# suvajit-patra/sl-hwgat

Measured on AMD Instinct MI355X. Metric: clips/sec fwd+bwd at B=64 T=128 J=67; %HBM roofline; 1->8 GPU scaling, higher is better.
Workload: dtype f32

## Files before the change

### sl-hwgat_amd/csrc/gemm_f32.h

```cpp
#pragma once
#include "common.h"

struct NtArgs {
    const float* A; const float* W; const float* bias; float* C;
    float* C2; const float* res; const float* aux;
    const float* mean; const float* rstd; const float* gamma; const float* beta;
    int64_t M; int N, K;
    uint32_t pro_seed, epi_seed; float pro_p, epi_p;
    int64_t row0;
    float* stat_sum; float* stat_sq;
    int mg_F, mg_K;
    const uint32_t* seed_base;
};

struct MergeWalk {
    int k, f; int64_t b; int F, K, step;
    __device__ __forceinline__ void start(int64_t m, int F_, int K_, int step_) {
        F = F_; K = K_; step = step_;
        const uint32_t mm = (uint32_t)m, fr = mm / (uint32_t)K_;
        k = (int)(mm - fr * (uint32_t)K_);
        const uint32_t bb = fr / (uint32_t)F_;
        f = (int)(fr - bb * (uint32_t)F_);
        b = bb;
    }
    __device__ __forceinline__ int64_t mrow() const { return (b * (F >> 1) + (f >> 1)) * K + k; }
    __device__ __forceinline__ int64_t off(int N) const { return mrow() * (2 * (int64_t)N) + (int64_t)(f & 1) * N; }
    __device__ __forceinline__ void next() {
        k += step;
        const bool wk = k >= K;
        k -= wk ? K : 0;
        f += wk ? 1 : 0;
        const bool wf = f >= F;
        f -= wf ? F : 0;
        b += wf ? 1 : 0;
    }
};

struct TnArgs {
    const float* A; const float* B; float* dW; float* db;
    const float* mean; const float* rstd; const float* gamma; const float* beta;
    int64_t M; int N, K;
    int n_split; int64_t rows_per_split;
    uint32_t pro_seed; float pro_p;
    int64_t row0;
    const uint32_t* seed_base;
    float* det_dw; float* det_db; int det_cap;
};


int hwgat_launch_tn256(TnArgs a, hipStream_t st, float* ws = nullptr, int64_t ws_floats = 0);
int64_t hwgat_tn256_ws_floats(int64_t M, int N, int K);

int hwgat_launch_nt256(const NtArgs& a, int pro, int epi, hipStream_t st);
```

### sl-hwgat_amd/csrc/gemm_f32.hip

```cpp
#include <stdlib.h>
#include <type_traits>
#include "common.h"
#include "fused_ops.h"
#include "gemm_f32.h"
#include "gemm_tn64.h"

namespace {

constexpr int BK_MIN = 16;

using NtSmall = TileCfg<2, 2, 2, 2>;
using NtBig = TileCfg<4, 2, 2, 4, 32, 1>;
using NtK16 = TileCfg<2, 2, 2, 2, 16, 3>;
using NtN64 = TileCfg<4, 1, 1, 2>;

template <int PRO, int EPI, typename C, bool RAGGED = false, int STAT = 0>
__global__ __launch_bounds__(C::THREADS, C::OCC * C::THREADS / 256) void gemm_nt_k(NtArgs p) {
    HWGAT_RESOLVE_SEEDS2(p);
    constexpr int BM = C::BM, BN = C::BN, TMW = C::TMW, TNW = C::TNW, PA = C::PA, PW = C::PW, RPP = C::RPP;
    constexpr int BK = C::BK, LDT = C::LDT;
    __shared__ __attribute__((aligned(16))) float sm[2 * (BM + BN) * LDT];
    const int tid = threadIdx.x, lane = tid & 63, wave = tid >> 6;
    const int lq = lane & 31, hh = lane >> 5;
    const int wm = wave / C::WN, wn = wave % C::WN;
    const int tiles_n = p.N / BN;
    const int row_blocks = RAGGED ? (int)((p.M + BM - 1) / BM) : (int)(p.M / BM);
    const int n_tiles = row_blocks * tiles_n;
    const int64_t m_last = p.M - 1;
    const int n_slab = p.K / BK;
    const int lrow = tid / C::TPR, lc4 = (tid % C::TPR) * 4;
    const uint32_t pro_th = drop_thresh(p.pro_p);
    const float pro_sc = 1.0f / (1.0f - p.pro_p);

    f32x4 ra[PA], rw[PW];
    float ln_mean[PA], ln_rstd[PA];
    f32x4 ln_g, ln_b;

    const int swz_tiles = (row_blocks / 8) * 8 * tiles_n;
    auto tile_origin = [&](int t, int64_t& m0, int& n0) {
        int rb, nt;
        if (t < swz_tiles) {
            rb = (t / (8 * tiles_n)) * 8 + (t & 7);
            nt = (t >> 3) % tiles_n;
        } else {
            const int w = t - swz_tiles;
            rb = (row_blocks / 8) * 8 + w / tiles_n;
            nt = w % tiles_n;
        }
        m0 = (int64_t)rb * BM;
        n0 = nt * BN;
    };
    auto issue = [&](int64_t m0, int n0, int slab, bool new_tile) {
        const int k0 = slab * BK + lc4;
#pragma unroll
        for (int i = 0; i < PA; ++i) {
            int64_t row = m0 + lrow + RPP * i;
            if constexpr (RAGGED) row = row < m_last ? row : m_last;
            ra[i] = *reinterpret_cast<const f32x4*>(p.A + row * p.K + k0);
            if constexpr (PRO == PRO_LN) {
                if (new_tile) { ln_mean[i] = p.mean[row]; ln_rstd[i] = p.rstd[row]; }
            }
        }
#pragma unroll
        for (int i = 0; i < PW; ++i)
            rw[i] = *reinterpret_cast<const f32x4*>(p.W + (int64_t)(n0 + lrow + RPP * i) * p.K + k0);
        if constexpr (PRO == PRO_LN) {
            ln_g = *reinterpret_cast<const f32x4*>(p.gamma + k0);
            ln_b = *reinterpret_cast<const f32x4*>(p.beta + k0);
        }
    };
    auto commit = [&](int buf, int64_t m0, int slab) {
        float* As = sm + buf * ((BM + BN) * LDT);
        float* Ws = As + BM * LDT;
        const int k0 = slab * BK + lc4;
#pragma unroll
        for (int i = 0; i < PA; ++i) {
            f32x4 a = ra[i];
            if constexpr (PRO == PRO_LN) {
                a = (a - ln_mean[i]) * (ln_rstd[i] * ln_g) + ln_b;
            } else if constexpr (PRO == PRO_DROP) {
                if (pro_th) a *= drop_keep4(p.pro_seed, (uint64_t)((RAGGED ? p.row0 : 0) + m0 + lrow + RPP * i) * p.K + k0, pro_th, pro_sc);
            }
            *reinterpret_cast<f32x4*>(As + (lrow + RPP * i) * LDT + lc4) = a;
        }
#pragma unroll
        for (int i = 0; i < PW; ++i) *reinterpret_cast<f32x4*>(Ws + (lrow + RPP * i) * LDT + lc4) = rw[i];
    };

    int t = blockIdx.x;
    if (t >= n_tiles) return;
    int64_t m0; int n0;
    tile_origin(t, m0, n0);
    issue(m0, n0, 0, true);
    commit(0, m0, 0);
    __syncthreads();
    int buf = 0;

    while (true) {
        f32x16 acc[TMW][TNW];
#pragma unroll
        for (int i = 0; i < TMW; ++i)
#pragma unroll
            for (int j = 0; j < TNW; ++j)
#pragma unroll
                for (int e = 0; e < 16; ++e) acc[i][j][e] = 0.f;

        int tn = t; int64_t mn = m0; int nn = n0;
        for (int s = 0; s < n_slab; ++s) {
            bool have_next = true, new_tile = false;
            int s_next = s + 1;
            if (s_next == n_slab) {
                tn = t + gridDim.x;
                have_next = tn < n_tiles;
                s_next = 0;
                new_tile = true;
                if (have_next) tile_origin(tn, mn, nn);
            }
            if (have_next) issue(mn, nn, s_next, new_tile);

            const float* As = sm + buf * ((BM + BN) * LDT);
            const float* Ws = As + BM * LDT;
            const float* ap = As + (wm * (TMW * 32) + lq) * LDT + 4 * hh;
            const float* wp = Ws + (wn * (TNW * 32) + lq) * LDT + 4 * hh;
#pragma unroll
            for (int kk = 0; kk < BK / 8; ++kk) {
                f32x4 af[TMW], bf[TNW];
#pragma unroll
                for (int i = 0; i < TMW; ++i) af[i] = *reinterpret_cast<const f32x4*>(ap + i * 32 * LDT + 8 * kk);
#pragma unroll
                for (int j = 0; j < TNW; ++j) bf[j] = *reinterpret_cast<const f32x4*>(wp + j * 32 * LDT + 8 * kk);
#pragma unroll
                for (int e = 0; e < 4; ++e)
#pragma unroll
                    for (int i = 0; i < TMW; ++i)
#pragma unroll
                        for (int j = 0; j < TNW; ++j)
                            acc[i][j] = __builtin_amdgcn_mfma_f32_32x32x2f32(af[i][e], bf[j][e], acc[i][j], 0, 0, 0);
            }
            if (have_next) commit(buf ^ 1, mn, s_next);
            __syncthreads();
            buf ^= 1;
        }

        {
            const uint32_t epi_th = drop_thresh(p.epi_p);
            const float epi_sc = 1.0f / (1.0f - p.epi_p);
            constexpr int SW = ((BM + BN) * LDT >= (C::THREADS / 64) * 32 * 68) ? 64 : 32;
            constexpr int SLD = SW + 4, LPR = SW / 4, RPS = 64 / LPR, NPS = 32 / RPS;
            float* stg = sm + (buf ^ 1) * ((BM + BN) * LDT) + wave * (32 * SLD);
            const int er = lane / LPR, ec = (lane % LPR) * 4;
            float* rowstat = sm + (buf ^ 1) * ((BM + BN) * LDT) + (C::THREADS / 64) * (32 * SLD);
            if constexpr (STAT == X_STAT || STAT == X_STAT_MERGE) {
                static_assert((C::THREADS / 64) * 32 * SLD + 2 * BM <= (BM + BN) * LDT, "no room for the row statistics");
                for (int q = tid; q < 2 * BM; q += C::THREADS) rowstat[q] = 0.f;
                __syncthreads();
            }
#pragma unroll
            for (int jc = 0; jc < TNW * 32 / SW; ++jc) {
                const int col = n0 + wn * (TNW * 32) + jc * SW + ec;
                f32x4 bv = {0.f, 0.f, 0.f, 0.f};
                if constexpr (epi_has_bias(EPI))
                    if (p.bias) bv = *reinterpret_cast<const f32x4*>(p.bias + col);
                f32x4 sv = bv, cv = bv;
                if constexpr (STAT == X_LNFOLD) {
                    sv = *reinterpret_cast<const f32x4*>(p.gamma + col);
                    cv = *reinterpret_cast<const f32x4*>(p.beta + col);
                }
#pragma unroll
                for (int i = 0; i < TMW; ++i) {
                    float rr_[NPS], rm[NPS];
                    if constexpr (STAT == X_LNFOLD) {
#pragma unroll
                        for (int ps = 0; ps < NPS; ++ps) {
                            int64_t grow = m0 + wm * (TMW * 32) + i * 32 + ps * RPS + er;
                            if constexpr (RAGGED) grow = grow < m_last ? grow : m_last;
                            rr_[ps] = p.rstd[grow]; rm[ps] = p.mean[grow];
                        }
                    }
                    MergeWalk mw;
                    if constexpr (STAT == X_STAT_MERGE) mw.start(m0 + wm * (TMW * 32) + i * 32 + er, p.mg_F, p.mg_K, RPS);
                    f32x4 ex[NPS];
                    if constexpr (epi_reads_extra(EPI)) {
                        const float* src = EPI == EPI_BIAS_DROP_RES ? p.res : p.aux;
#pragma unroll
                        for (int ps = 0; ps < NPS; ++ps) {
                            int64_t grow = m0 + wm * (TMW * 32) + i * 32 + ps * RPS + er;
                            if constexpr (RAGGED) grow = grow < m_last ? grow : m_last;
                            ex[ps] = *reinterpret_cast<const f32x4*>(src + grow * p.N + col);
                        }
                    }
#pragma unroll
                    for (int j = 0; j < SW / 32; ++j)
#pragma unroll
                        for (int r = 0; r < 16; ++r)
                            stg[crow(r, hh) * SLD + j * 32 + lq] = acc[i][jc * (SW / 32) + j][r];
                    __builtin_amdgcn_fence(__ATOMIC_ACQ_REL, "wavefront");
                    __builtin_amdgcn_wave_barrier();
#pragma unroll
                    for (int ps = 0; ps < NPS; ++ps) {
                        const int rr = ps * RPS + er;
                        const int64_t grow = m0 + wm * (TMW * 32) + i * 32 + rr;
                        if constexpr (RAGGED) { if (grow > m_last) continue; }
                        const int64_t off = grow * p.N + col;
                        f32x4 v = *reinterpret_cast<const f32x4*>(stg + rr * SLD + ec);
                        if constexpr (STAT == X_LNFOLD) v = v * rr_[ps] + (cv - sv * (rm[ps] * rr_[ps]));
                        else v += bv;
                        f32x4 dk = {1.f, 1.f, 1.f, 1.f};
                        if constexpr (epi_drops(EPI)) {
                            if (epi_th) dk = drop_keep4(p.epi_seed, (uint64_t)(off + (RAGGED ? p.row0 * p.N : 0)), epi_th, epi_sc);
                        }
                        if constexpr (EPI == EPI_BIAS_DROP_RES) {
                            v = ex[ps] + v * dk;
                        } else if constexpr (EPI == EPI_BIAS_GELU_DROP) {
                            *reinterpret_cast<f32x4*>(p.C2 + off) = v;
                            v.x = gelu_f(v.x) * dk.x; v.y = gelu_f(v.y) * dk.y;
                            v.z = gelu_f(v.z) * dk.z; v.w = gelu_f(v.w) * dk.w;
                        } else if constexpr (EPI == EPI_BIAS_GELU_DROP_G) {
                            float u4[4] = {v.x, v.y, v.z, v.w}, g4[4];
                            const float k4[4] = {dk.x, dk.y, dk.z, dk.w};
#pragma unroll
                            for (int e = 0; e < 4; ++e) gelu_fwd_grad(u4[e], k4[e], u4[e], g4[e]);
                            v = f32x4{u4[0], u4[1], u4[2], u4[3]};
                            const f32x4 gq = {g4[0], g4[1], g4[2], g4[3]};
                            *reinterpret_cast<f32x4*>(p.C2 + off) = gq;
                        } else if constexpr (EPI == EPI_MUL_AUX) {
                            v *= ex[ps];
                        } else if constexpr (EPI == EPI_BIAS_RELU_DROP) {
                            v.x = fmaxf(v.x, 0.f) * dk.x; v.y = fmaxf(v.y, 0.f) * dk.y;
                            v.z = fmaxf(v.z, 0.f) * dk.z; v.w = fmaxf(v.w, 0.f) * dk.w;
                        } else if constexpr (EPI == EPI_RELU_BWD) {
                            const f32x4 u = ex[ps];
                            v.x *= u.x > 0.f ? epi_sc : 0.f; v.y *= u.y > 0.f ? epi_sc : 0.f;
                            v.z *= u.z > 0.f ? epi_sc : 0.f; v.w *= u.w > 0.f ? epi_sc : 0.f;
                        } else if constexpr (EPI == EPI_GELU_BWD) {
                            const f32x4 h = ex[ps];
                            v.x *= dk.x * gelu_grad(h.x); v.y *= dk.y * gelu_grad(h.y);
                            v.z *= dk.z * gelu_grad(h.z); v.w *= dk.w * gelu_grad(h.w);
                        }
                        if constexpr (STAT == X_STAT || STAT == X_STAT_MERGE) {
                            float s1 = (v.x + v.y) + (v.z + v.w), s2 = (v.x * v.x + v.y * v.y) + (v.z * v.z + v.w * v.w);
                            s1 = group_sum<LPR>(s1); s2 = group_sum<LPR>(s2);
                            if ((lane % LPR) == 0) {
                                const int lr = wm * (TMW * 32) + i * 32 + rr;
                                atomicAdd(rowstat + 2 * lr, s1);
                                atomicAdd(rowstat + 2 * lr + 1, s2);
                            }
                            if constexpr (STAT == X_STAT_MERGE) {
                                *reinterpret_cast<f32x4*>(p.C + mw.off(p.N) + col) = v;
                                mw.next();
                            } else {
                                *reinterpret_cast<f32x4*>(p.C + off) = v;
                            }
                        } else {
                            *reinterpret_cast<f32x4*>(p.C + off) = v;
                        }
                    }
                    __builtin_amdgcn_fence(__ATOMIC_ACQ_REL, "wavefront");
                    __builtin_amdgcn_wave_barrier();
                }
            }
            if constexpr (STAT == X_STAT || STAT == X_STAT_MERGE) {
                __syncthreads();
                for (int q = tid; q < BM; q += C::THREADS) {
                    int64_t mr = m0 + q;
                    if constexpr (STAT == X_STAT_MERGE) { MergeWalk w; w.start(m0 + q, p.mg_F, p.mg_K, 1); mr = w.mrow(); }
                    atomicAdd(p.stat_sum + mr, rowstat[2 * q]);
                    atomicAdd(p.stat_sq + mr, rowstat[2 * q + 1]);
                }
            }
        }
        __syncthreads();
        t += gridDim.x;
        if (t >= n_tiles) break;
        m0 = mn; n0 = nn;
    }
}


using TnSmall = TileCfg<2, 2, 2, 2>;
using TnBig = TileCfg<4, 2, 2, 4, 32, 1>;
using TnK16 = TileCfg<2, 2, 2, 2, 16, 3>;

template <int PRO, bool BLN, typename C, bool MF16 = false, bool RAGGED = false>
__global__ __launch_bounds__(C::THREADS, C::OCC * C::THREADS / 256) void gemm_tn_k(TnArgs p) {
    HWGAT_RESOLVE_SEED1(p);
    constexpr int TM = C::BK;
    constexpr int BT = C::BM;
    constexpr int LDR = MF16 ? BT + 16 : BT;
    constexpr int TNW = C::TMW, TKW = C::TNW;
    constexpr int TPR = BT / 4;
    constexpr int RPP = C::THREADS / TPR;
    constexpr int NP = TM / RPP;
    __shared__ __attribute__((aligned(16))) float sm[2 * 2 * TM * LDR];
    const int tid = threadIdx.x, lane = tid & 63, wave = tid >> 6;
    const int lq = lane & 31, hh = lane >> 5;
    const int wn = wave / C::WN, wk = wave % C::WN;
    const int tiles_n = p.N / BT, tiles_k = p.K / BT, n_tiles = tiles_n * tiles_k;
    const int xcd = blockIdx.x & 7, j = blockIdx.x >> 3;
    const int tile = j % n_tiles;
    const int split = (j / n_tiles) * 8 + xcd;
    if (split >= p.n_split) return;
    const int n0 = (tile / tiles_k) * BT, k0 = (tile % tiles_k) * BT;
    const int64_t r_begin = (int64_t)split * p.rows_per_split;
    const int64_t r_end = r_begin + p.rows_per_split < p.M ? r_begin + p.rows_per_split : p.M;
    if (r_begin >= r_end) return;
    const int n_it = RAGGED ? (int)((r_end - r_begin + TM - 1) / TM) : (int)((r_end - r_begin) / TM);
    const int64_t m_last = p.M - 1;

    const int lrow = tid / TPR, lc4 = (tid % TPR) * 4;
    const uint32_t pro_th = drop_thresh(p.pro_p);
    const float pro_sc = 1.0f / (1.0f - p.pro_p);
    f32x4 ra[NP], rb[NP];
    float bm[NP], bs[NP];
    f32x4 colsum = {0.f, 0.f, 0.f, 0.f};
    f32x4 lg = {1.f, 1.f, 1.f, 1.f}, lb = {0.f, 0.f, 0.f, 0.f};
    if constexpr (BLN) {
        lg = *reinterpret_cast<const f32x4*>(p.gamma + k0 + lc4);
        lb = *reinterpret_cast<const f32x4*>(p.beta + k0 + lc4);
    }

    auto issue = [&](int it) {
        const int64_t r0 = r_begin + (int64_t)it * TM + lrow;
#pragma unroll
        for (int i = 0; i < NP; ++i) {
            int64_t row = r0 + RPP * i;
            if constexpr (RAGGED) row = row < m_last ? row : m_last;
            ra[i] = *reinterpret_cast<const f32x4*>(p.A + row * p.N + n0 + lc4);
            rb[i] = *reinterpret_cast<const f32x4*>(p.B + row * p.K + k0 + lc4);
            if constexpr (BLN) { bm[i] = p.mean[row]; bs[i] = p.rstd[row]; }
        }
    };
    auto commit = [&](int buf, int it) {
        float* As = sm + buf * (2 * TM * LDR);
        float* Bs = As + TM * LDR;
        const int64_t r0 = r_begin + (int64_t)it * TM + lrow;
#pragma unroll
        for (int i = 0; i < NP; ++i) {
            f32x4 a = ra[i], b = rb[i];
            if constexpr (PRO == PRO_DROP)
                a *= drop_keep4(p.pro_seed, (uint64_t)((RAGGED ? p.row0 : 0) + r0 + RPP * i) * p.N + n0 + lc4, pro_th, pro_sc);
            if constexpr (BLN) b = (b - bm[i]) * bs[i] * lg + lb;
            if constexpr (RAGGED) { if (r0 + RPP * i > m_last) a = f32x4{0.f, 0.f, 0.f, 0.f}; }
            colsum += a;
            *reinterpret_cast<f32x4*>(As + (lrow + RPP * i) * LDR + lc4) = a;
            *reinterpret_cast<f32x4*>(Bs + (lrow + RPP * i) * LDR + lc4) = b;
        }
    };

    constexpr int TI = MF16 ? TNW * 2 : TNW, TJ = MF16 ? TKW * 2 : TKW, TS = MF16 ? 16 : 32;
    typedef typename std::conditional<MF16, f32x4, f32x16>::type acc_t;
    acc_t acc[TI][TJ];
#pragma unroll
    for (int i = 0; i < TI; ++i)
#pragma unroll
        for (int jj = 0; jj < TJ; ++jj)
#pragma unroll
            for (int e = 0; e < (MF16 ? 4 : 16); ++e) acc[i][jj][e] = 0.f;

    issue(0);
    commit(0, 0);
    __syncthreads();
    int buf = 0;
    const int lc = MF16 ? (lane & 15) : lq, lk = MF16 ? (lane >> 4) : hh;
    constexpr int KPS = MF16 ? 4 : 2;
    for (int it = 0; it < n_it; ++it) {
        const bool have_next = it + 1 < n_it;
        if (have_next) issue(it + 1);
        const float* As = sm + buf * (2 * TM * LDR) + wn * (TNW * 32) + lc;
        const float* Bs = sm + buf * (2 * TM * LDR) + TM * LDR + wk * (TKW * 32) + lc;
        constexpr int NSTEP = TM / KPS, CH = MF16 ? 2 : 4, NCH = NSTEP / CH;
        float fa[2][CH][TI], fb[2][CH][TJ];
        auto fetch = [&](int c, int slot) {
#pragma unroll
            for (int e = 0; e < CH; ++e) {
                const int ro = (KPS * (c * CH + e) + lk) * LDR;
#pragma unroll
                for (int i = 0; i < TI; ++i) fa[slot][e][i] = As[ro + TS * i];
#pragma unroll
                for (int jj = 0; jj < TJ; ++jj) fb[slot][e][jj] = Bs[ro + TS * jj];
            }
        };
        fetch(0, 0);
#pragma unroll
        for (int c = 0; c < NCH; ++c) {
            if (c + 1 < NCH) fetch(c + 1, (c + 1) & 1);
            __builtin_amdgcn_sched_barrier(0);
#pragma unroll
            for (int e = 0; e < CH; ++e)
#pragma unroll
                for (int i = 0; i < TI; ++i)
#pragma unroll
                    for (int jj = 0; jj < TJ; ++jj) {
                        if constexpr (MF16)
                            acc[i][jj] = __builtin_amdgcn_mfma_f32_16x16x4f32(fa[c & 1][e][i], fb[c & 1][e][jj], acc[i][jj], 0, 0, 0);
                        else
                            acc[i][jj] = __builtin_amdgcn_mfma_f32_32x32x2f32(fa[c & 1][e][i], fb[c & 1][e][jj], acc[i][jj], 0, 0, 0);
                    }
            __builtin_amdgcn_sched_barrier(0);
        }
        if (have_next) commit(buf ^ 1, it + 1);
        __syncthreads();
        buf ^= 1;
    }
    const bool det = p.det_dw != nullptr;
    float* dwo = det ? p.det_dw + (int64_t)split * p.N * p.K : p.dW;
#pragma unroll
    for (int i = 0; i < TI; ++i)
#pragma unroll
        for (int jj = 0; jj < TJ; ++jj)
#pragma unroll
            for (int r = 0; r < (MF16 ? 4 : 16); ++r) {
                const int n = n0 + wn * (TNW * 32) + i * TS + (MF16 ? 4 * lk + r : crow(r, hh));
                const int k = k0 + wk * (TKW * 32) + jj * TS + lc;
                HWGAT_TN_ACC(det, dwo, (int64_t)n * p.K + k, acc[i][jj][r]);
            }
    if (p.db != nullptr && k0 == 0) {
        float* red = sm;
        __syncthreads();
        *reinterpret_cast<f32x4*>(red + lrow * BT + lc4) = colsum;
        __syncthreads();
        if (tid < BT) {
            float s = 0.f;
#pragma unroll
            for (int q = 0; q < RPP; ++q) s += red[q * BT + tid];
            HWGAT_TN_ACC(det, det ? p.det_db + (int64_t)split * p.N : p.db, n0 + tid, s);
        }
    }
}

__global__ void transpose_k(const float* __restrict__ in, float* __restrict__ out, int R, int C) {
    __shared__ float tile[32][33];
    const int c0 = blockIdx.x * 32, r0 = blockIdx.y * 32;
    for (int i = threadIdx.y; i < 32; i += 8)
        if (r0 + i < R && c0 + threadIdx.x < C) tile[i][threadIdx.x] = in[(int64_t)(r0 + i) * C + c0 + threadIdx.x];
    __syncthreads();
    for (int i = threadIdx.y; i < 32; i += 8)
        if (c0 + i < C && r0 + threadIdx.x < R) out[(int64_t)(c0 + i) * R + r0 + threadIdx.x] = tile[threadIdx.x][i];
}

template <int PRO, typename C, bool RAGGED = false>
int launch_nt(const NtArgs& a, int epi, hipStream_t st, bool fold = false) {
    const int64_t tiles = ((a.M + C::BM - 1) / C::BM) * (a.N / C::BN);
    const int grid = (int)(tiles < C::SLOTS ? tiles : C::SLOTS);
    if (fold) {
        if constexpr (PRO == PRO_NONE) {
            if (epi == EPI_BIAS) gemm_nt_k<PRO_NONE, EPI_BIAS, C, RAGGED, X_LNFOLD><<<grid, C::THREADS, 0, st>>>(a);
            else if (epi == EPI_BIAS_GELU_DROP) gemm_nt_k<PRO_NONE, EPI_BIAS_GELU_DROP, C, RAGGED, X_LNFOLD><<<grid, C::THREADS, 0, st>>>(a);
            else if (epi == EPI_BIAS_GELU_DROP_G) gemm_nt_k<PRO_NONE, EPI_BIAS_GELU_DROP_G, C, RAGGED, X_LNFOLD><<<grid, C::THREADS, 0, st>>>(a);
            else return HWGAT_EINVAL;
            HWGAT_LAUNCH_CHECK();
        }
        return HWGAT_EINVAL;
    }
    if (a.stat_sum != nullptr) {
        if constexpr (PRO == PRO_NONE && !RAGGED) {
            if (a.mg_K > 0) gemm_nt_k<PRO_NONE, EPI_BIAS_DROP_RES, C, false, 2><<<grid, C::THREADS, 0, st>>>(a);
            else gemm_nt_k<PRO_NONE, EPI_BIAS_DROP_RES, C, false, 1><<<grid, C::THREADS, 0, st>>>(a);
            HWGAT_LAUNCH_CHECK();
        }
        return HWGAT_EINVAL;
    }
    switch (epi) {
        case EPI_BIAS: gemm_nt_k<PRO, EPI_BIAS, C, RAGGED><<<grid, C::THREADS, 0, st>>>(a); break;
        case EPI_BIAS_DROP_RES: gemm_nt_k<PRO, EPI_BIAS_DROP_RES, C, RAGGED><<<grid, C::THREADS, 0, st>>>(a); break;
        case EPI_BIAS_GELU_DROP: gemm_nt_k<PRO, EPI_BIAS_GELU_DROP, C, RAGGED><<<grid, C::THREADS, 0, st>>>(a); break;
        case EPI_GELU_BWD: gemm_nt_k<PRO, EPI_GELU_BWD, C, RAGGED><<<grid, C::THREADS, 0, st>>>(a); break;
        case EPI_BIAS_GELU_DROP_G: gemm_nt_k<PRO, EPI_BIAS_GELU_DROP_G, C, RAGGED><<<grid, C::THREADS, 0, st>>>(a); break;
        case EPI_MUL_AUX: gemm_nt_k<PRO, EPI_MUL_AUX, C, RAGGED><<<grid, C::THREADS, 0, st>>>(a); break;
        case EPI_NONE: gemm_nt_k<PRO, EPI_NONE, C, RAGGED><<<grid, C::THREADS, 0, st>>>(a); break;
        case EPI_BIAS_RELU_DROP:
            if constexpr (PRO == PRO_NONE) { gemm_nt_k<PRO_NONE, EPI_BIAS_RELU_DROP, C, RAGGED><<<grid, C::THREADS, 0, st>>>(a); break; }
            return HWGAT_EINVAL;
        case EPI_RELU_BWD:
            if constexpr (PRO == PRO_NONE) { gemm_nt_k<PRO_NONE, EPI_RELU_BWD, C, RAGGED><<<grid, C::THREADS, 0, st>>>(a); break; }
            return HWGAT_EINVAL;
        default: return HWGAT_EINVAL;
    }
    HWGAT_LAUNCH_CHECK();
}

NtArgs nt_rows(NtArgs a, int64_t r0, int64_t rows) {
    a.A += r0 * a.K;
    a.C += r0 * a.N;
    if (a.C2) a.C2 += r0 * a.N;
    if (a.res) a.res += r0 * a.N;
    if (a.aux) a.aux += r0 * a.N;
    if (a.mean) { a.mean += r0; a.rstd += r0; }
    a.M = rows;
    a.row0 = r0;
    return a;
}
TnArgs tn_rows(TnArgs a, int64_t r0, int64_t rows) {
    a.A += r0 * a.N;
    a.B += r0 * a.K;
    if (a.mean) { a.mean += r0; a.rstd += r0; }
    a.M = rows;
    a.row0 = r0;
    return a;
}

int tile_override() {
    static const int v = [] {
        const char* e = lab_env("HWGAT_GEMM_TILE");
        return !e ? 0 : (e[0] == 's' ? 1 : (e[0] == 'b' ? 2 : (e[0] == 'k' ? 3 : (e[0] == 'm' ? 6 : (e[0] == 't' ? 7 : 0)))));
    }();
    return v;
}

int launch_nt_n64(const NtArgs& a, int pro, int epi, hipStream_t st) {
    const int64_t m_bulk = a.M / 128 * 128;
    if (m_bulk) {
        NtArgs b = a;
        b.M = m_bulk;
        int rc;
        switch (pro) {
            case PRO_NONE: rc = launch_nt<PRO_NONE, NtN64>(b, epi, st); break;
            case PRO_LN_FOLD: rc = launch_nt<PRO_NONE, NtN64>(b, epi, st, true); break;
            case PRO_LN: rc = launch_nt<PRO_LN, NtN64>(b, epi, st); break;
            case PRO_DROP: rc = launch_nt<PRO_DROP, NtN64>(b, epi, st); break;
            default: return HWGAT_EINVAL;
        }
        if (rc || m_bulk == a.M) return rc;
    }
    const NtArgs t = nt_rows(a, m_bulk, a.M - m_bulk);
    switch (pro) {
        case PRO_NONE: return launch_nt<PRO_NONE, NtN64, true>(t, epi, st);
        case PRO_LN: return launch_nt<PRO_LN, NtN64, true>(t, epi, st);
        case PRO_DROP: return launch_nt<PRO_DROP, NtN64, true>(t, epi, st);
        default: return HWGAT_EINVAL;
    }
}

template <int PRO, bool BLN, typename C, bool MF16 = false, bool RAGGED = false>
int launch_tn(TnArgs a, hipStream_t st) {
    constexpr int TM = C::BK;
    const int n_tiles = (a.N / C::BM) * (a.K / C::BM);
    auto gcd = [](int x, int y) { while (y) { int t = x % y; x = y; y = t; } return x; };
    const int r_min = n_tiles / gcd(n_tiles, C::SLOTS);
    static const int min_rounds = [] { const char* e = lab_env("HWGAT_TN_ROUNDS"); return e ? atoi(e) : 1; }();
    int r = r_min;
    while (r < min_rounds) r += r_min;
    int64_t want = (int64_t)C::SLOTS * r / n_tiles;
    const int64_t max_split = a.M / (TM * 16) > 0 ? a.M / (TM * 16) : 1;
    if (want > max_split) want = max_split;
    if (want < 1) want = 1;
    int64_t rows = (a.M + want - 1) / want;
    rows = (rows + TM - 1) / TM * TM;
    a.n_split = (int)((a.M + rows - 1) / rows);
    a.rows_per_split = rows;
    if (a.det_dw && a.n_split > a.det_cap) return HWGAT_ESHAPE;
    const int grid = ((a.n_split + 7) / 8) * 8 * n_tiles;
    gemm_tn_k<PRO, BLN, C, MF16, RAGGED><<<grid, C::THREADS, 0, st>>>(a);
    HWGAT_LAUNCH_CHECK();
}

}

extern "C" int hwgat_linear_nt_f32_ex(const float* A, const float* W, const float* bias, float* C, int64_t M,
                                      int N, int K, int pro, const float* mean, const float* rstd,
                                      const float* gamma, const float* beta, uint32_t pro_seed, float pro_p,
                                      int epi, const float* res, float* C2, const float* aux, uint32_t epi_seed,
                                      float epi_p, float* stat_sum, float* stat_sq, int merge_F, int merge_K,
                                      const uint32_t* seed_base, void* stream) {
    if (!A || !W || !C || M <= 0 || N <= 0 || K <= 0) return HWGAT_EINVAL;
    if (N % 64 || K % 32 || ((M + 127) / 128) * (int64_t)(N / 64) > 0x7fffffff) return HWGAT_ESHAPE;
    if ((pro == PRO_LN || pro == PRO_LN_FOLD) && (!mean || !rstd || !gamma || !beta)) return HWGAT_EINVAL;
    if (pro == PRO_LN_FOLD) {
        if (epi != EPI_BIAS && epi != EPI_BIAS_GELU_DROP && epi != EPI_BIAS_GELU_DROP_G) return HWGAT_EINVAL;
        if (M % 128) return HWGAT_ESHAPE;
    }
    if (epi == EPI_BIAS_DROP_RES && !res) return HWGAT_EINVAL;
    if ((epi == EPI_BIAS_GELU_DROP || epi == EPI_BIAS_GELU_DROP_G) && !C2) return HWGAT_EINVAL;
    if ((epi == EPI_GELU_BWD || epi == EPI_MUL_AUX || epi == EPI_RELU_BWD) && !aux) return HWGAT_EINVAL;
    if (pro_p < 0.f || pro_p >= 1.f || epi_p < 0.f || epi_p >= 1.f) return HWGAT_EINVAL;
    if (epi_is_relu(epi) && pro != PRO_NONE) return HWGAT_EINVAL;
    const bool stat = stat_sum != nullptr || stat_sq != nullptr || merge_K > 0;
    if (stat) {
        if (!stat_sum || !stat_sq || pro != PRO_NONE || epi != EPI_BIAS_DROP_RES) return HWGAT_EINVAL;
        if (M % 256) return HWGAT_ESHAPE;
        if (merge_K > 0 && (merge_F <= 0 || (merge_F & 1) || M % ((int64_t)merge_F * merge_K))) return HWGAT_EINVAL;
    }
    if (pro == PRO_DROP && pro_p == 0.f) pro = PRO_NONE;
    NtArgs a{A, W, bias, C, C2, res, aux, mean, rstd, gamma, beta, M, N, K, pro_seed, epi_seed, pro_p, epi_p, 0, stat_sum, stat_sq, merge_K > 0 ? merge_F : 0, merge_K > 0 ? merge_K : 0};
    a.seed_base = seed_base;
    hipStream_t st = (hipStream_t)stream;
    if (N % 128) {
        if (stat) return HWGAT_ESHAPE;
        return launch_nt_n64(a, pro, epi, st);
    }
    const int64_t m_bulk = M / 128 * 128;
    if (m_bulk != M) {
        if (m_bulk) {
            const int rc = hwgat_linear_nt_f32(A, W, bias, C, m_bulk, N, K, pro, mean, rstd, gamma, beta, pro_seed, pro_p,
                                               epi, res, C2, aux, epi_seed, epi_p, seed_base, stream);
            if (rc) return rc;
        }
        const NtArgs t = nt_rows(a, m_bulk, M - m_bulk);
        switch (pro) {
            case PRO_NONE: return launch_nt<PRO_NONE, NtSmall, true>(t, epi, st);
            case PRO_LN: return launch_nt<PRO_LN, NtSmall, true>(t, epi, st);
            case PRO_DROP: return launch_nt<PRO_DROP, NtSmall, true>(t, epi, st);
            default: return HWGAT_EINVAL;
        }
    }
    static const bool nt_old = [] { const char* e = lab_env("HWGAT_NT_KERNEL"); return e && e[0] == 'o'; }();
    static const int nt256_min_k = [] { const char* e = lab_env("HWGAT_NT256_MINK"); return e ? atoi(e) : 128; }();
    if (!nt_old && !epi_is_relu(epi) && tile_override() == 0 && N % 256 == 0 && K >= nt256_min_k && M >= 256 &&
        ((M / 256) * (N / 256) >= 128 || a.stat_sum != nullptr)) {
        const int64_t m256 = M / 256 * 256;
        NtArgs b = a;
        b.M = m256;
        const int rc = hwgat_launch_nt256(b, pro, epi, st);
        if (rc || m256 == M) return rc;
        const NtArgs t = nt_rows(a, m256, M - m256);
        switch (pro) {
            case PRO_NONE: return launch_nt<PRO_NONE, NtSmall, true>(t, epi, st);
            case PRO_LN_FOLD: return launch_nt<PRO_NONE, NtSmall, true>(t, epi, st, true);
            case PRO_LN: return launch_nt<PRO_LN, NtSmall, true>(t, epi, st);
            case PRO_DROP: return launch_nt<PRO_DROP, NtSmall, true>(t, epi, st);
            default: return HWGAT_EINVAL;
        }
    }
    const bool heavy = epi == EPI_BIAS_DROP_RES || epi == EPI_BIAS_GELU_DROP || epi == EPI_GELU_BWD || epi == EPI_BIAS_GELU_DROP_G || epi == EPI_MUL_AUX ||
                       epi_is_relu(epi);
    const bool big = tile_override() == 2 && (M % 256 == 0) && (N % 256 == 0);
    const bool k16 = tile_override() == 3 || (tile_override() == 0 && heavy);
#define NT_GO(P) return big ? launch_nt<P, NtBig>(a, epi, st) : (k16 ? launch_nt<P, NtK16>(a, epi, st) : launch_nt<P, NtSmall>(a, epi, st))
    switch (pro) {
        case PRO_NONE: NT_GO(PRO_NONE);
        case PRO_LN_FOLD: return k16 ? launch_nt<PRO_NONE, NtK16>(a, epi, st, true) : launch_nt<PRO_NONE, NtSmall>(a, epi, st, true);
        case PRO_LN: NT_GO(PRO_LN);
        case PRO_DROP: NT_GO(PRO_DROP);
        default: return HWGAT_EINVAL;
    }
#undef NT_GO
}

extern "C" int hwgat_linear_nt_f32(const float* A, const float* W, const float* bias, float* C, int64_t M,
                                   int N, int K, int pro, const float* mean, const float* rstd,
                                   const float* gamma, const float* beta, uint32_t pro_seed, float pro_p,
                                   int epi, const float* res, float* C2, const float* aux, uint32_t epi_seed,
                                   float epi_p, const uint32_t* seed_base, void* stream) {
    return hwgat_linear_nt_f32_ex(A, W, bias, C, M, N, K, pro, mean, rstd, gamma, beta, pro_seed, pro_p, epi, res, C2, aux,
                                  epi_seed, epi_p, nullptr, nullptr, 0, 0, seed_base, stream);
}

static bool tn256_takes(int64_t M, int N, int K, float pro_p, const float* mean) {
    const int ov = tile_override();
    return M % 32 == 0 && (ov == 0 || ov == 7) && N % 256 == 0 && K % 256 == 0 && (int64_t)N * K > 256 * 256 && !(pro_p > 0.f && mean);
}

extern "C" int64_t hwgat_linear_tn_f32_ws_bytes(int64_t M, int N, int K) {
    if (hwgat_tn64_takes(N, K)) return hwgat_tn64_ws_bytes(M, N, K);
    if (M <= 0 || N <= 0 || K <= 0 || !tn256_takes(M, N, K, 0.f, nullptr)) return 0;
    return hwgat_tn256_ws_floats(M, N, K) * 4;
}

extern "C" int hwgat_linear_tn_f32_ws(const float* A, const float* B, float* dW, float* db, int64_t M, int N,
                                      int K, uint32_t pro_seed, float pro_p, const float* mean,
                                      const float* rstd, const float* gamma, const float* beta, float* ws,
                                      int64_t ws_bytes, const uint32_t* seed_base, void* stream) {
    if (!A || !B || !dW || M <= 0 || N <= 0 || K <= 0) return HWGAT_EINVAL;
    if (mean && (!rstd || !gamma || !beta)) return HWGAT_EINVAL;
    if (pro_p < 0.f || pro_p >= 1.f) return HWGAT_EINVAL;
    if (hwgat_tn64_takes(N, K))
        return hwgat_tn64_run(HWGAT_F32, A, B, dW, db, M, N, K, pro_seed, pro_p, mean, rstd, gamma, beta, seed_base,
                              ws && ws_bytes >= hwgat_tn64_ws_bytes(M, N, K) ? ws : nullptr, ws_bytes, (hipStream_t)stream);
    if (ws && ws_bytes > 0 && N % 128 == 0 && K % 128 == 0 && tn256_takes(M, N, K, pro_p, mean)) {
        TnArgs a{A, B, dW, db, mean, rstd, gamma, beta, M, N, K, 0, 0, pro_seed, pro_p, 0};
        a.seed_base = seed_base;
        return hwgat_launch_tn256(a, (hipStream_t)stream, ws, ws_bytes / 4);
    }
    return hwgat_linear_tn_f32(A, B, dW, db, M, N, K, pro_seed, pro_p, mean, rstd, gamma, beta, seed_base, stream);
}

static int tn_f32_impl(const float* A, const float* B, float* dW, float* db, int64_t M, int N,
                       int K, uint32_t pro_seed, float pro_p, const float* mean,
                       const float* rstd, const float* gamma, const float* beta,
                       const uint32_t* seed_base, DetWs det, void* stream) {
    if (!A || !B || !dW || M <= 0 || N <= 0 || K <= 0) return HWGAT_EINVAL;
    if (mean && (!rstd || !gamma || !beta)) return HWGAT_EINVAL;
    if (N % 128 || K % 128) return HWGAT_ESHAPE;
    if (pro_p < 0.f || pro_p >= 1.f) return HWGAT_EINVAL;
    TnArgs a{A, B, dW, db, mean, rstd, gamma, beta, M, N, K, 0, 0, pro_seed, pro_p, 0};
    a.seed_base = seed_base;
    a.det_dw = det.dw; a.det_db = det.db; a.det_cap = det.cap;
    hipStream_t st = (hipStream_t)stream;
    const int64_t m_bulk = M / 32 * 32;
    if (m_bulk != M) {
        if (det.dw) return HWGAT_ESHAPE;
        if (m_bulk) {
            const int rc = hwgat_linear_tn_f32(A, B, dW, db, m_bulk, N, K, pro_seed, pro_p, mean, rstd, gamma, beta, seed_base, stream);
            if (rc) return rc;
        }
        const TnArgs t = tn_rows(a, m_bulk, M - m_bulk);
        if (pro_p > 0.f) return mean ? launch_tn<PRO_DROP, true, TnSmall, false, true>(t, st) : launch_tn<PRO_DROP, false, TnSmall, false, true>(t, st);
        return mean ? launch_tn<PRO_NONE, true, TnSmall, false, true>(t, st) : launch_tn<PRO_NONE, false, TnSmall, false, true>(t, st);
    }
    const int ov = tile_override();
    if ((ov == 0 || ov == 7) && N % 256 == 0 && K % 256 == 0 && (int64_t)N * K > 256 * 256 && !(pro_p > 0.f && mean))
        return hwgat_launch_tn256(a, st);
    const bool big = ov == 2 && (N % 256 == 0) && (K % 256 == 0);
    const bool k16 = ov == 3;
    const bool mf16 = ov == 6;
#define TN_GO(P, L) return mf16 ? launch_tn<P, L, TnSmall, true>(a, st) : (big ? launch_tn<P, L, TnBig>(a, st) : (k16 ? launch_tn<P, L, TnK16>(a, st) : launch_tn<P, L, TnSmall>(a, st)))
    if (pro_p > 0.f) { if (mean) TN_GO(PRO_DROP, true); else TN_GO(PRO_DROP, false); }
    if (mean) TN_GO(PRO_NONE, true);
    TN_GO(PRO_NONE, false);
#undef TN_GO
}

extern "C" int hwgat_linear_tn_f32(const float* A, const float* B, float* dW, float* db, int64_t M, int N,
                                   int K, uint32_t pro_seed, float pro_p, const float* mean,
                                   const float* rstd, const float* gamma, const float* beta,
                                   const uint32_t* seed_base, void* stream) {
    if (hwgat_tn64_takes(N, K))
        return hwgat_tn64_run(HWGAT_F32, A, B, dW, db, M, N, K, pro_seed, pro_p, mean, rstd, gamma, beta, seed_base,
                              nullptr, 0, (hipStream_t)stream);
    return tn_f32_impl(A, B, dW, db, M, N, K, pro_seed, pro_p, mean, rstd, gamma, beta, seed_base, DetWs{nullptr, nullptr, 0}, stream);
}

namespace {
__global__ __launch_bounds__(256) void tn_det_reduce_k(const float* __restrict__ ws, float* __restrict__ out, int cap, int64_t stride,
                                                       int64_t count) {
    const int64_t i = (int64_t)blockIdx.x * 256 + threadIdx.x;
    if (i >= count) return;
    float s = 0.f;
    int sp = 0;
    for (; sp + 8 <= cap; sp += 8) {
        float v[8];
#pragma unroll
        for (int j = 0; j < 8; ++j) v[j] = ws[(sp + j) * stride + i];
#pragma unroll
        for (int j = 0; j < 8; ++j) s += v[j];
    }
    for (; sp < cap; ++sp) s += ws[sp * stride + i];
    out[i] += s;
}
}
int hwgat_tn_det_reduce(const float* ws, float* out, int cap, int64_t stride, int64_t count, hipStream_t st) {
    tn_det_reduce_k<<<(unsigned)((count + 255) / 256), 256, 0, st>>>(ws, out, cap, stride, count);
    HWGAT_LAUNCH_CHECK();
}

static int64_t tn_det_cap(int64_t M, int N, int K) {
    auto gcd = [](int64_t x, int64_t y) { while (y) { int64_t t = x % y; x = y; y = t; } return x; };
    const int64_t t128 = (int64_t)(N / 128) * (K / 128);
    int64_t cap = 0;
    for (int64_t slots : {512, 768, 1024}) {
        const int64_t r = t128 / gcd(t128, slots);
        cap = cap > slots * r / t128 ? cap : slots * r / t128;
    }
    if (N % 256 == 0 && K % 256 == 0) {
        const int64_t t256 = (int64_t)(N / 256) * (K / 256), r = t256 / gcd(t256, 256);
        const int64_t w = 256 * r / t256 > 8 ? 256 * r / t256 : 8;
        cap = cap > w ? cap : w;
    }
    const int64_t by_rows = M / 32 + 1;
    cap = cap < by_rows ? cap : by_rows;
    return cap + 8;
}
extern "C" int64_t hwgat_linear_tn_det_bytes(int64_t M, int N, int K) {
    if (hwgat_tn64_takes(N, K)) return hwgat_tn64_ws_bytes(M, N, K);
    if (M <= 0 || N <= 0 || K <= 0 || N % 128 || K % 128) return 0;
    return tn_det_cap(M, N, K) * ((int64_t)N * K + N) * 4;
}

extern "C" int hwgat_linear_tn_f32_det(const float* A, const float* B, float* dW, float* db, int64_t M, int N,
                                       int K, uint32_t pro_seed, float pro_p, const float* mean,
                                       const float* rstd, const float* gamma, const float* beta,
                                       const uint32_t* seed_base, float* ws, int64_t ws_bytes, void* stream) {
    if (!ws || N <= 0 || K <= 0) return HWGAT_EINVAL;
    if (hwgat_tn64_takes(N, K))
        return hwgat_tn64_run(HWGAT_F32, A, B, dW, db, M, N, K, pro_seed, pro_p, mean, rstd, gamma, beta, seed_base, ws,
                              ws_bytes, (hipStream_t)stream);
    const int64_t per = (int64_t)N * K + N;
    const int64_t cap = ws_bytes / 4 / per;
    if (cap < 1) return HWGAT_ESHAPE;
    const DetWs det{ws, ws + cap * (int64_t)N * K, (int)(cap > 0x7fffffff ? 0x7fffffff : cap)};
    int rc = tn_f32_impl(A, B, dW, db, M, N, K, pro_seed, pro_p, mean, rstd, gamma, beta, seed_base, det, stream);
    if (rc) return rc;
    rc = hwgat_tn_det_reduce(det.dw, dW, det.cap, (int64_t)N * K, (int64_t)N * K, (hipStream_t)stream);
    if (rc || !db) return rc;
    return hwgat_tn_det_reduce(det.db, db, det.cap, N, N, (hipStream_t)stream);
}

extern "C" int hwgat_transpose_f32(const float* in, float* out, int R, int C, void* stream) {
    if (!in || !out || R <= 0 || C <= 0) return HWGAT_EINVAL;
    dim3 grid((C + 31) / 32, (R + 31) / 32), block(32, 8);
    transpose_k<<<grid, block, 0, (hipStream_t)stream>>>(in, out, R, C);
    HWGAT_LAUNCH_CHECK();
}

__global__ void drop_mask_k(float* out, int64_t n, uint32_t seed, float p, const uint32_t* seed_base) {
    seed += seed_base_of(seed_base);
    const uint32_t th = drop_thresh(p);
    const float sc = 1.0f / (1.0f - p);
    for (int64_t i = (int64_t)blockIdx.x * 256 + threadIdx.x; i < n; i += (int64_t)gridDim.x * 256)
        out[i] = drop_keep(seed, (uint64_t)i, th, sc);
}
extern "C" int hwgat_dropout_mask_f32(float* out, int64_t n, uint32_t seed, float p, const uint32_t* seed_base, void* stream) {
    if (!out || n <= 0 || p < 0.f || p >= 1.f) return HWGAT_EINVAL;
    const int grid = (int)((n + 255) / 256 < 2048 ? (n + 255) / 256 : 2048);
    drop_mask_k<<<grid, 256, 0, (hipStream_t)stream>>>(out, n, seed, p, seed_base);
    HWGAT_LAUNCH_CHECK();
}
```

Measured before the change: 635.4.

## Add split-K MFMA weight-gradient GEMM for shapes with a 128 dimension

Adds a dedicated TN GEMM path for weight gradients where N or K equals 128 (both at most 1024). It splits the M (row) dimension across about 256 blocks. Each block runs a software-pipelined loop of 32x32x2 f32 MFMA instructions with four register buffers and explicit scheduling-group hints, then reduces its partial tile across waves in LDS and writes it to a workspace slab. A second kernel sums the slabs into dW and db. The aim is to fill the GPU on these narrow weight-gradient GEMMs, which otherwise launch too few tiles, at the cost of extra workspace memory traffic and one more kernel launch.

```diff
diff --git a/sl-hwgat_amd/csrc/gemm_f32.h b/sl-hwgat_amd/csrc/gemm_f32.h
--- a/sl-hwgat_amd/csrc/gemm_f32.h
+++ b/sl-hwgat_amd/csrc/gemm_f32.h
@@ -51,4 +51,8 @@
 int hwgat_launch_tn256(TnArgs a, hipStream_t st, float* ws = nullptr, int64_t ws_floats = 0);
 int64_t hwgat_tn256_ws_floats(int64_t M, int N, int K);
 
+bool hwgat_tn128_takes(int64_t M, int N, int K, float pro_p, const float* mean);
+int64_t hwgat_tn128_ws_floats(int64_t M, int N, int K);
+int hwgat_launch_tn128(TnArgs a, hipStream_t st, float* ws, int64_t ws_floats);
+
 int hwgat_launch_nt256(const NtArgs& a, int pro, int epi, hipStream_t st);
diff --git a/sl-hwgat_amd/csrc/gemm_f32.hip b/sl-hwgat_amd/csrc/gemm_f32.hip
--- a/sl-hwgat_amd/csrc/gemm_f32.hip
+++ b/sl-hwgat_amd/csrc/gemm_f32.hip
@@ -652,6 +652,7 @@
 
 extern "C" int64_t hwgat_linear_tn_f32_ws_bytes(int64_t M, int N, int K) {
     if (hwgat_tn64_takes(N, K)) return hwgat_tn64_ws_bytes(M, N, K);
+    if (tile_override() == 0 && hwgat_tn128_takes(M, N, K, 0.f, nullptr)) return hwgat_tn128_ws_floats(M, N, K) * 4;
     if (M <= 0 || N <= 0 || K <= 0 || !tn256_takes(M, N, K, 0.f, nullptr)) return 0;
     return hwgat_tn256_ws_floats(M, N, K) * 4;
 }
@@ -666,6 +667,11 @@
     if (hwgat_tn64_takes(N, K))
         return hwgat_tn64_run(HWGAT_F32, A, B, dW, db, M, N, K, pro_seed, pro_p, mean, rstd, gamma, beta, seed_base,
                               ws && ws_bytes >= hwgat_tn64_ws_bytes(M, N, K) ? ws : nullptr, ws_bytes, (hipStream_t)stream);
+    if (ws && tile_override() == 0 && hwgat_tn128_takes(M, N, K, pro_p, mean) && ws_bytes / 4 >= hwgat_tn128_ws_floats(M, N, K)) {
+        TnArgs a{A, B, dW, db, mean, rstd, gamma, beta, M, N, K, 0, 0, pro_seed, pro_p, 0};
+        a.seed_base = seed_base;
+        return hwgat_launch_tn128(a, (hipStream_t)stream, ws, ws_bytes / 4);
+    }
     if (ws && ws_bytes > 0 && N % 128 == 0 && K % 128 == 0 && tn256_takes(M, N, K, pro_p, mean)) {
         TnArgs a{A, B, dW, db, mean, rstd, gamma, beta, M, N, K, 0, 0, pro_seed, pro_p, 0};
         a.seed_base = seed_base;
diff --git a/sl-hwgat_amd/csrc/gemm_f32_tn128.hip b/sl-hwgat_amd/csrc/gemm_f32_tn128.hip
--- /dev/null
+++ b/sl-hwgat_amd/csrc/gemm_f32_tn128.hip
@@ -0,0 +1,222 @@
+#include <stdlib.h>
+#include <type_traits>
+#include "common.h"
+#include "fused_ops.h"
+#include "gemm_f32.h"
+
+namespace {
+
+constexpr int SLAB = 16384 + 128;
+constexpr int SG_VALU = 0x002, SG_MFMA = 0x008, SG_VMEM_RD = 0x020;
+
+struct RegSet { f32x4 a[4], b[4], mu, rs; };
+
+__device__ __forceinline__ int slab_pos(int t, int q, int lane) { return ((t * 4 + q) * 64 + lane) * 4; }
+
+template <int PRO, bool BLN>
+__global__ __launch_bounds__(256, 1) void gemm_tn128_k(TnArgs p, float* __restrict__ ws) {
+    HWGAT_RESOLVE_SEED1(p);
+    __shared__ __attribute__((aligned(16))) float red[2 * 16384];
+    __shared__ __attribute__((aligned(16))) float bsum[4 * 128];
+    const int tid = threadIdx.x, lane = tid & 63, wave = tid >> 6;
+    const int lq = lane & 31, hh = lane >> 5;
+    const int tiles_k = p.K / 128, n_tiles = (p.N / 128) * tiles_k;
+    const int L = (blockIdx.x & 7) * (int)(gridDim.x >> 3) + (int)(blockIdx.x >> 3);
+    if (L >= p.n_split * n_tiles) return;
+    const int split = L / n_tiles, tile = L % n_tiles;
+    const int n0 = (tile / tiles_k) * 128, k0 = (tile % tiles_k) * 128;
+    const int64_t r_begin = (int64_t)split * p.rows_per_split;
+    const int64_t r_end = r_begin + p.rows_per_split < p.M ? r_begin + p.rows_per_split : p.M;
+    const int G = (int)((r_end - r_begin) >> 5);
+    const int64_t row_l = r_begin + 8 * wave + 4 * hh;
+    const float* Ap = p.A + row_l * p.N + n0 + 4 * lq;
+    const float* Bp = p.B + row_l * p.K + k0 + 4 * lq;
+    const uint32_t pro_th = drop_thresh(p.pro_p);
+    const float pro_sc = 1.0f / (1.0f - p.pro_p);
+    f32x4 lg = {1.f, 1.f, 1.f, 1.f}, lb = {0.f, 0.f, 0.f, 0.f};
+    if constexpr (BLN) {
+        lg = *reinterpret_cast<const f32x4*>(p.gamma + k0 + 4 * lq);
+        lb = *reinterpret_cast<const f32x4*>(p.beta + k0 + 4 * lq);
+    }
+    f32x4 colsum = {0.f, 0.f, 0.f, 0.f};
+
+    RegSet S[4];
+    auto load = [&](RegSet& r, int u) {
+        const int64_t ro = 32 * (int64_t)u;
+#pragma unroll
+        for (int s = 0; s < 4; ++s) {
+            r.a[s] = *reinterpret_cast<const f32x4*>(Ap + (ro + s) * p.N);
+            r.b[s] = *reinterpret_cast<const f32x4*>(Bp + (ro + s) * p.K);
+        }
+        if constexpr (BLN) {
+            r.mu = *reinterpret_cast<const f32x4*>(p.mean + row_l + ro);
+            r.rs = *reinterpret_cast<const f32x4*>(p.rstd + row_l + ro);
+        }
+    };
+    auto prep = [&](RegSet& r, int u, float live) {
+#pragma unroll
+        for (int s = 0; s < 4; ++s) {
+            if constexpr (PRO == PRO_DROP)
+                r.a[s] *= drop_keep4(p.pro_seed, (uint64_t)(row_l + 32 * (int64_t)u + s) * p.N + n0 + 4 * lq, pro_th, pro_sc);
+            if constexpr (BLN) r.b[s] = (r.b[s] - r.mu[s]) * r.rs[s] * lg + lb;
+            colsum += r.a[s] * live;
+        }
+    };
+
+    f32x16 acc[4][4];
+#pragma unroll
+    for (int i = 0; i < 4; ++i)
+#pragma unroll
+        for (int j = 0; j < 4; ++j)
+#pragma unroll
+            for (int e = 0; e < 16; ++e) acc[i][j][e] = 0.f;
+
+    auto mfma = [&](const RegSet& r) {
+#pragma unroll
+        for (int s = 0; s < 4; ++s)
+#pragma unroll
+            for (int i = 0; i < 4; ++i)
+#pragma unroll
+                for (int j = 0; j < 4; ++j)
+                    acc[i][j] = __builtin_amdgcn_mfma_f32_32x32x2f32(r.a[s][i], r.b[s][j], acc[i][j], 0, 0, 0);
+    };
+    auto body = [&](auto QC, int u) {
+        constexpr int Q = decltype(QC)::value;
+        load(S[(Q + 2) & 3], u + 2 < G ? u + 2 : G - 1);
+        mfma(S[Q]);
+        prep(S[(Q + 1) & 3], u + 1, u + 1 < G ? 1.f : 0.f);
+        __builtin_amdgcn_sched_group_barrier(SG_VMEM_RD, BLN ? 10 : 8, 0);
+#pragma unroll
+        for (int q = 0; q < 16; ++q) {
+            __builtin_amdgcn_sched_group_barrier(SG_MFMA, 4, 0);
+            __builtin_amdgcn_sched_group_barrier(SG_VALU, 6, 0);
+        }
+        __builtin_amdgcn_sched_barrier(0);
+    };
+    using Q0 = std::integral_constant<int, 0>;
+    using Q1 = std::integral_constant<int, 1>;
+    using Q2 = std::integral_constant<int, 2>;
+    using Q3 = std::integral_constant<int, 3>;
+    load(S[0], 0);
+    load(S[1], 1 < G ? 1 : G - 1);
+    prep(S[0], 0, 1.f);
+    for (int u = 0; u < G; u += 4) {
+        body(Q0{}, u);
+        body(Q1{}, u + 1);
+        body(Q2{}, u + 2);
+        body(Q3{}, u + 3);
+    }
+
+    auto park = [&](float* dst) {
+#pragma unroll
+        for (int t = 0; t < 16; ++t)
+#pragma unroll
+            for (int q = 0; q < 4; ++q) {
+                const f32x16& v = acc[t >> 2][t & 3];
+                *reinterpret_cast<f32x4*>(dst + slab_pos(t, q, lane)) = f32x4{v[4 * q], v[4 * q + 1], v[4 * q + 2], v[4 * q + 3]};
+            }
+    };
+    auto take = [&](const float* src) {
+#pragma unroll
+        for (int t = 0; t < 16; ++t)
+#pragma unroll
+            for (int q = 0; q < 4; ++q) {
+                const f32x4 v = *reinterpret_cast<const f32x4*>(src + slab_pos(t, q, lane));
+#pragma unroll
+                for (int e = 0; e < 4; ++e) acc[t >> 2][t & 3][4 * q + e] += v[e];
+            }
+    };
+    colsum.x += __shfl_xor(colsum.x, 32);
+    colsum.y += __shfl_xor(colsum.y, 32);
+    colsum.z += __shfl_xor(colsum.z, 32);
+    colsum.w += __shfl_xor(colsum.w, 32);
+    if (hh == 0) *reinterpret_cast<f32x4*>(bsum + wave * 128 + 4 * lq) = colsum;
+    if (wave >= 2) park(red + (wave - 2) * 16384);
+    __syncthreads();
+    if (wave < 2) take(red + wave * 16384);
+    __syncthreads();
+    if (wave == 1) park(red);
+    __syncthreads();
+    if (wave != 0) return;
+    take(red);
+    float* slab = ws + (int64_t)L * SLAB;
+#pragma unroll
+    for (int t = 0; t < 16; ++t)
+#pragma unroll
+        for (int q = 0; q < 4; ++q) {
+            const f32x16& v = acc[t >> 2][t & 3];
+            *reinterpret_cast<f32x4*>(slab + slab_pos(t, q, lane)) = f32x4{v[4 * q], v[4 * q + 1], v[4 * q + 2], v[4 * q + 3]};
+        }
+    if (p.db != nullptr && k0 == 0) {
+#pragma unroll
+        for (int c = 0; c < 2; ++c) {
+            const int col = c * 64 + lane;
+            slab[16384 + col] = ((bsum[col] + bsum[128 + col]) + bsum[256 + col]) + bsum[384 + col];
+        }
+    }
+}
+
+__global__ __launch_bounds__(256) void tn128_reduce_k(const float* __restrict__ ws, float* __restrict__ dW, float* __restrict__ db,
+                                                      int n_split, int n_tiles, int tiles_k, int K) {
+    const int tile = blockIdx.x / 65;
+    const int idx = (blockIdx.x % 65) * 256 + threadIdx.x;
+    if (idx >= SLAB) return;
+    const int n0 = (tile / tiles_k) * 128, k0 = (tile % tiles_k) * 128;
+    if (idx >= 16384 && (db == nullptr || k0 != 0)) return;
+    const float* src = ws + (int64_t)tile * SLAB + idx;
+    const int64_t step = (int64_t)n_tiles * SLAB;
+    float s = 0.f;
+    int sp = 0;
+    for (; sp + 8 <= n_split; sp += 8) {
+        float v[8];
+#pragma unroll
+        for (int j = 0; j < 8; ++j) v[j] = src[(sp + j) * step];
+#pragma unroll
+        for (int j = 0; j < 8; ++j) s += v[j];
+    }
+    for (; sp < n_split; ++sp) s += src[sp * step];
+    if (idx >= 16384) {
+        db[n0 + idx - 16384] += s;
+        return;
+    }
+    const int e = idx & 3, lane = (idx >> 2) & 63, q = (idx >> 8) & 3, t = idx >> 10;
+    const int i = t >> 2, j = t & 3, lq = lane & 31, hh = lane >> 5;
+    dW[(int64_t)(n0 + 4 * crow(4 * q + e, hh) + i) * K + k0 + 4 * lq + j] += s;
+}
+
+void tn128_split(int64_t M, int n_tiles, int& n_split, int64_t& rows_per_split) {
+    const int64_t want = 256 / n_tiles;
+    int64_t rows = (M + want - 1) / want;
+    rows = (rows + 127) / 128 * 128;
+    n_split = (int)((M + rows - 1) / rows);
+    rows_per_split = rows;
+}
+
+}
+
+bool hwgat_tn128_takes(int64_t M, int N, int K, float pro_p, const float* mean) {
+    return M > 0 && M % 128 == 0 && N % 128 == 0 && K % 128 == 0 && (N == 128 || K == 128) && N <= 1024 && K <= 1024 &&
+           !(pro_p > 0.f && mean);
+}
+
+int64_t hwgat_tn128_ws_floats(int64_t M, int N, int K) {
+    if (!hwgat_tn128_takes(M, N, K, 0.f, nullptr)) return 0;
+    const int n_tiles = (N / 128) * (K / 128);
+    int n_split;
+    int64_t rows;
+    tn128_split(M, n_tiles, n_split, rows);
+    return (int64_t)n_split * n_tiles * SLAB;
+}
+
+int hwgat_launch_tn128(TnArgs a, hipStream_t st, float* ws, int64_t ws_floats) {
+    if (!ws || !hwgat_tn128_takes(a.M, a.N, a.K, a.pro_p, a.mean)) return HWGAT_ESHAPE;
+    const int n_tiles = (a.N / 128) * (a.K / 128);
+    tn128_split(a.M, n_tiles, a.n_split, a.rows_per_split);
+    if (ws_floats < (int64_t)a.n_split * n_tiles * SLAB) return HWGAT_ESHAPE;
+    const int grid = (a.n_split * n_tiles + 7) / 8 * 8;
+    if (a.pro_p > 0.f) gemm_tn128_k<PRO_DROP, false><<<grid, 256, 0, st>>>(a, ws);
+    else if (a.mean) gemm_tn128_k<PRO_NONE, true><<<grid, 256, 0, st>>>(a, ws);
+    else gemm_tn128_k<PRO_NONE, false><<<grid, 256, 0, st>>>(a, ws);
+    tn128_reduce_k<<<n_tiles * 65, 256, 0, st>>>(ws, a.dW, a.db, a.n_split, n_tiles, a.K / 128, a.K);
+    HWGAT_LAUNCH_CHECK();
+}
```

Result: no change. 637.7 (median of 6 runs) (+0.4%).
